# Tarseus/eam-rl4co

Hardware: AMD Instinct MI355X
Metric: env-steps/sec (batch x num_loc / s), AttentionModel construction rollout (higher is better)
Workload: dtype f32; 1 GPU; TSP num_loc=100 batch=1024/GPU AM greedy rollout (encoder + cache + decode loop + reward); global_batch=1024, launch=hipGraph replay

## Files before the change

eam_rl4co_amd/_lib.py:

```python
from __future__ import annotations

import ctypes as C
import os

_PKG = os.path.dirname(os.path.abspath(__file__))
LIB_PATH = os.environ.get("EAMRL_HIP_LIB") or os.path.join(_PKG, "lib", "libeamrl_hip.so")

ENV_TSP, ENV_CVRP, ENV_SDVRP, ENV_PCTSP, ENV_OP, ENV_CVRPTW, ENV_PDP = 0, 1, 2, 3, 4, 5, 6
GREEDY, SAMPLE, EVALUATE = 0, 1, 2
NORM_BATCH_EVAL, NORM_INSTANCE = 0, 1
ST_NAN_LOGITS, ST_INFEASIBLE, ST_STEP_OVERRUN = 1, 2, 4
LINEAR_NONE = 0

_vp, _i64, _i32, _f32 = C.c_void_p, C.c_int64, C.c_int, C.c_float


class Cache(C.Structure):
    _fields_ = [("K", _vp), ("V", _vp), ("Lp", _vp), ("Pa", _vp), ("Pb", _vp), ("cvec", _vp), ("gctx", _vp),
                ("ld", _i64), ("B", _i64), ("M", C.c_int32), ("E", C.c_int32), ("H", C.c_int32),
                ("dyn", _vp)]


class EncoderLayer(C.Structure):
    _fields_ = [(n, _vp) for n in ("Wqkv", "bqkv", "Wo", "bo", "W1", "b1", "W2", "b2", "n1_gamma", "n1_beta", "n1_mean",
                                   "n1_var", "n2_gamma", "n2_beta", "n2_mean", "n2_var")]


class EncoderCache(C.Structure):
    _fields_ = [("Wc", _vp), ("WoutT", _vp), ("out", _vp), ("ld", _i64), ("nproj", C.c_int32), ("Wg", _vp), ("gctx", _vp)]


class EncoderInit(C.Structure):
    _fields_ = [("feat", _vp), ("F", C.c_int32), ("W", _vp), ("b", _vp), ("depot", _vp), ("depot_ld", _i64), ("Wd", _vp),
                ("bd", _vp), ("init_out", _vp)]


class Reeval(C.Structure):
    _fields_ = [("K", _vp), ("V", _vp), ("Lp", _vp), ("Pa", _vp), ("Pb", _vp), ("ld", _i64),
                ("gctx", _vp), ("Cvec", _vp), ("NC", C.c_int32),
                ("idxA", _vp), ("idxB", _vp), ("sc", _vp), ("maskbits", _vp), ("actions", _vp),
                ("B", _i64), ("R", _i64), ("S", C.c_int32), ("T", C.c_int32), ("M", C.c_int32), ("tstart", C.c_int32),
                ("nchunk", C.c_int32), ("clip", _f32), ("temp", _f32),
                ("logp", _vp), ("lse", _vp), ("glogp", _vp), ("dheads", _vp), ("heads", _vp), ("heads_T", C.c_int32),
                ("entropy", _vp),
# ... 157 lines not shown
```

eam_rl4co_amd/csrc/abi.hip:

```cpp
#include <cstdarg>
#include <cstdio>

#include "kernels.hpp"


using namespace eamrl;

namespace eamrl { int g_debug[16] = {0}; }

static thread_local char g_err[256] = "";

static int fail(int code, const char* fmt, ...)
{
    va_list ap;
    va_start(ap, fmt);
    vsnprintf(g_err, sizeof(g_err), fmt, ap);
    va_end(ap);
    return code;
}

static int launched(int rc, const char* what)
{
    if (rc == 0) return 0;
    if (rc == EAMRL_E_ARG) return fail(rc, "%s: unsupported shape", what);
// ... 378 lines not shown
    REQUIRE(xy && code && out && R >= 0 && B > 0 && N > 0, "eamrl_augment_xy");
    REQUIRE(((uintptr_t)xy % 8 == 0) && ((uintptr_t)out % 8 == 0), "eamrl_augment_xy");
    return launched(launch_augment_xy(xy, cs, code, out, R, B, N, offset, (hipStream_t)stream), "eamrl_augment_xy");
}

static bool dtype16_ok(int dtype) { return dtype == EAMRL_DTYPE_F16 || dtype == EAMRL_DTYPE_BF16; }

static int encoder_fused_entry(const float* h_in, const eamrl_encoder_init* init, bool with_init, float* h_out, int64_t B, int M,
                               int E, int H, int ff_hidden, int nlayers, int norm, float eps, const eamrl_encoder_layer* layers,
                               const eamrl_encoder_cache* cache, int dtype, void* stream, const char* what)
{
    if (cache) {
        REQUIRE(cache->Wc && cache->WoutT && cache->out && cache->nproj >= 3 && cache->nproj <= 5, what);
        REQUIRE(cache->ld >= (int64_t)(cache->nproj + 1) * E && cache->ld % 4 == 0 && ((uintptr_t)cache->out % 16 == 0) &&
                    ((uintptr_t)cache->Wc % 16 == 0) && ((uintptr_t)cache->WoutT % 16 == 0), what);
    }
    REQUIRE(layers && B >= 0, what);
    REQUIRE(encoder_fused_supports(M, E, H, ff_hidden, nlayers), what);
    REQUIRE(norm == EAMRL_NORM_BATCH_EVAL || norm == EAMRL_NORM_INSTANCE, what);
    for (int l = 0; l < nlayers; ++l) {
        const eamrl_encoder_layer& s = layers[l];
        REQUIRE(s.Wqkv && s.bqkv && s.Wo && s.bo && s.W1 && s.b1 && s.W2 && s.b2 && s.n1_gamma && s.n1_beta && s.n2_gamma &&
                    s.n2_beta, what);
        REQUIRE(((uintptr_t)s.Wqkv % 16 == 0) && ((uintptr_t)s.Wo % 16 == 0) && ((uintptr_t)s.W1 % 16 == 0) &&
                    ((uintptr_t)s.W2 % 16 == 0), what);
        if (norm == EAMRL_NORM_BATCH_EVAL) REQUIRE(s.n1_mean && s.n1_var && s.n2_mean && s.n2_var, what);
    }
    if (with_init) {
        REQUIRE(init && init->feat && init->W && init->F >= 1 && init->F <= 8, what);
        REQUIRE(!init->depot || (init->Wd && init->depot_ld >= 2), what);
// ... 200 lines not shown
    REQUIRE(x && dy && mean && rstd && dx && B >= 0 && N > 0 && E > 0, "eamrl_instance_norm_backward");
    if (B == 0) return 0;
    return launched(launch_instnorm_train_bwd(x, dy, mean, rstd, gamma, dx, dgamma, dbeta, B, N, E, (hipStream_t)stream),
                    "eamrl_instance_norm_backward");
}

__attribute__((visibility("default"))) int eamrl_mean_nodes(const float* emb, float* out, int64_t B, int M, int E,
                                                           void* stream)
{
    REQUIRE(emb && out && B >= 0 && M > 0 && E > 0, "eamrl_mean_nodes");
    return launched(launch_mean_nodes(emb, out, B, M, E, (hipStream_t)stream), "eamrl_mean_nodes");
}

static int fill_args(const char* what, int env, const eamrl_cache* c, const eamrl_state* s, int64_t R, int mode,
                     const float* noise, const int64_t* given, float clip, float temp, int top_k, double top_p,
                     uint32_t* status, DecArgs& a, bool seeded = false)
{
    REQUIRE(c && s, what);
    REQUIRE(env >= EAMRL_ENV_TSP && env <= EAMRL_ENV_PDP, what);
    REQUIRE(mode == EAMRL_GREEDY || mode == EAMRL_SAMPLE || mode == EAMRL_EVALUATE, what);
    REQUIRE(c->K && c->V && c->Lp && c->Pa && (c->cvec || env == EAMRL_ENV_PDP), what);
    REQUIRE(c->B > 0 && c->M > 0 && c->E > 0 && c->H > 0, what);
    REQUIRE(c->E % c->H == 0 && (c->E / c->H) % 4 == 0 && c->E % (4 * EAMRL_NCHUNK) == 0, what);
    REQUIRE(c->ld >= c->E && c->ld % 4 == 0, what);
    REQUIRE(((uintptr_t)c->K % 16 == 0) && ((uintptr_t)c->V % 16 == 0) && ((uintptr_t)c->Lp % 16 == 0), what);
    REQUIRE(R > 0 && R % c->B == 0 && R <= 0x7fffffffLL, what);
    REQUIRE(s->cur && s->mask && status, what);
    REQUIRE(temp > 0.0f && top_k >= 0 && top_p >= 0.0 && top_p <= 1.0, what);
    if (env == EAMRL_ENV_TSP) REQUIRE(c->Pb && s->first && s->istep, what);
    if (env == EAMRL_ENV_CVRP) REQUIRE(s->used && s->vcap && c->M >= 2, what);
    if (env == EAMRL_ENV_SDVRP) REQUIRE(s->used && s->vcap && s->rem && c->dyn && c->M >= 2, what);
    if (env == EAMRL_ENV_PCTSP) REQUIRE(s->used && s->vcap && c->M >= 2, what);
    if (env == EAMRL_ENV_OP) REQUIRE(s->used && s->vcap && c->M >= 2, what);
    if (env == EAMRL_ENV_CVRPTW) REQUIRE(s->used && s->vcap && s->time && c->M >= 2, what);
    if (env == EAMRL_ENV_PDP) REQUIRE(c->M >= 3 && c->M % 2 == 1, what);
    if (mode == EAMRL_SAMPLE) REQUIRE(noise != nullptr || seeded, what);
    if (mode == EAMRL_EVALUATE) REQUIRE(given != nullptr, what);
    a = DecArgs{};
    a.K = c->K; a.V = c->V; a.Lp = c->Lp; a.Pa = c->Pa; a.Pb = c->Pb; a.cvec = c->cvec; a.gctx = c->gctx;
    a.ld = c->ld; a.B = c->B; a.M = c->M; a.E = c->E; a.H = c->H;
    a.first = s->first; a.cur = s->cur; a.istep = s->istep; a.used = s->used; a.vcap = s->vcap; a.demand = s->demand;
    a.mask = s->mask; a.visited = s->visited; a.done = s->done;
    a.rem = s->rem; a.dyn = c->dyn; a.locs = s->locs; a.time = s->time; a.tw = s->tw; a.dur = s->dur;
    a.heads_out = s->heads_out;
    a.to_deliver = s->to_deliver;
    a.seed = 0; a.seed_dev = nullptr; a.use_rng = 0;
    a.R = R; a.mode = mode; a.noise = noise; a.given = given; a.clip = clip; a.temp = temp; a.top_k = top_k; a.top_p = top_p; a.status = status;
    return 0;
}

__attribute__((visibility("default"))) int eamrl_am_decode_step(int env, const eamrl_cache* cache_host,
                                                               const eamrl_state* state_host, int64_t R, int mode,
                                                               const float* noise, const int64_t* given, float tanh_clip,
                                                               float temperature, int top_k, double top_p,
                                                               int fuse_env_step, int64_t* action,
                                                               float* logp, float* logprobs_all, float* logits_raw,
                                                               uint32_t* status, void* stream)
{
    DecArgs a;
    int rc = fill_args("eamrl_am_decode_step", env, cache_host, state_host, R, mode, noise, given, tanh_clip, temperature,
// ... 32 lines not shown
    DecArgs a{};
    a.B = cache_host->B; a.M = cache_host->M; a.E = cache_host->E; a.H = cache_host->H; a.ld = cache_host->ld; a.R = R;
    a.t_max = t_max; a.top_k = top_k; a.top_p = top_p;
    return rollout_kernel_for(env, a, true);
}

__attribute__((visibility("default"))) int eamrl_am_rollout(int env, const eamrl_cache* cache_host,
                                                           const eamrl_state* state_host, int64_t R, int mode,
                                                           const float* noise, const int64_t* given, int t_given,
                                                           float tanh_clip, float temperature, int top_k, double top_p,
                                                           int t_max, int64_t* actions, float* logps, int32_t* steps_out,
                                                           uint32_t* status, void* stream)
{
    DecArgs a;
    int rc = fill_args("eamrl_am_rollout", env, cache_host, state_host, R, mode, noise, given, tanh_clip, temperature,
                       top_k, top_p, status, a);
    if (rc) return rc;
    REQUIRE(actions && logps && steps_out && a.done && t_max > 0, "eamrl_am_rollout");
    if (env == EAMRL_ENV_CVRP) REQUIRE(a.visited && a.demand, "eamrl_am_rollout");
    if (env == EAMRL_ENV_PCTSP) REQUIRE(a.visited && a.demand && a.istep, "eamrl_am_rollout");
    if (env == EAMRL_ENV_OP) REQUIRE(a.visited && a.demand && a.istep && a.locs, "eamrl_am_rollout");
    if (env == EAMRL_ENV_CVRPTW) REQUIRE(a.visited && a.demand && a.locs && a.tw && a.dur, "eamrl_am_rollout");
    if (env == EAMRL_ENV_PDP) REQUIRE(a.visited && a.to_deliver, "eamrl_am_rollout");
    if (mode == EAMRL_EVALUATE) REQUIRE(t_given > 0, "eamrl_am_rollout");
    a.fuse_env = 1; a.t_max = t_max; a.t_given = t_given;
    a.action = actions; a.logp = logps; a.steps_out = steps_out;
    const int kernel = rollout_kernel_for(env, a, false);
    if (kernel == EAMRL_KERNEL_MS_MFMA)
        return launched(launch_rollout_ms_mfma(env, a, (hipStream_t)stream), "eamrl_am_rollout");
    if (kernel == EAMRL_KERNEL_RESIDENT)
        return launched(launch_rollout_resident(env, a, (hipStream_t)stream), "eamrl_am_rollout");
    return launched(launch_rollout_stream(env, a, (hipStream_t)stream), "eamrl_am_rollout");
}

__attribute__((visibility("default"))) int eamrl_exp1_noise(uint64_t seed, const uint64_t* seed_dev, float* noise, int64_t R,
                                                           int T, int M, void* stream)
{
    REQUIRE(noise && R >= 0 && T > 0 && M > 0, "eamrl_exp1_noise");
    return launched(launch_exp1_noise(seed, seed_dev, noise, R, T, M, (hipStream_t)stream), "eamrl_exp1_noise");
}

__attribute__((visibility("default"))) int eamrl_rollout_rng_native(int env, const eamrl_cache* cache_host, int64_t R)
// ... 1 lines not shown
    if (!cache_host || R <= 0 || g_debug[11]) return 0;
    DecArgs a{};
    a.B = cache_host->B; a.M = cache_host->M; a.E = cache_host->E; a.H = cache_host->H; a.ld = cache_host->ld; a.R = R;
    return rollout_ms_mfma_supports(env, a, true) ? 1 : 0;
}

__attribute__((visibility("default"))) int eamrl_am_rollout_seeded(int env, const eamrl_cache* cache_host,
                                                                  const eamrl_state* state_host, int64_t R, uint64_t seed,
                                                                  const uint64_t* seed_dev, float* noise_scratch,
                                                                  float tanh_clip, float temperature,
                                                                  int t_max, int64_t* actions, float* logps,
                                                                  int32_t* steps_out, uint32_t* status, void* stream)
{
    DecArgs a;
    int rc = fill_args("eamrl_am_rollout_seeded", env, cache_host, state_host, R, EAMRL_SAMPLE, nullptr, nullptr, tanh_clip,
                       temperature, 0, 0.0, status, a, true);
    if (rc) return rc;
    REQUIRE(actions && logps && steps_out && a.done && t_max > 0, "eamrl_am_rollout_seeded");
    a.fuse_env = 1; a.t_max = t_max; a.t_given = 0;
    a.action = actions; a.logp = logps; a.steps_out = steps_out;
    if (rollout_kernel_for(env, a, false) == EAMRL_KERNEL_MS_MFMA) {
        a.seed = seed; a.seed_dev = seed_dev; a.use_rng = 1;
        return launched(launch_rollout_ms_mfma(env, a, (hipStream_t)stream), "eamrl_am_rollout_seeded");
    }
    REQUIRE(noise_scratch != nullptr, "eamrl_am_rollout_seeded (noise_scratch [R][t_max][M] needed for this shape)");
    rc = launch_exp1_noise(seed, seed_dev, noise_scratch, R, t_max, a.M, (hipStream_t)stream);
    if (rc) return launched(rc, "eamrl_am_rollout_seeded");
    return eamrl_am_rollout(env, cache_host, state_host, R, EAMRL_SAMPLE, noise_scratch, nullptr, 0, tanh_clip, temperature, 0,
                            0.0, t_max, actions, logps, steps_out, status, stream);
}

static bool polynet_shape_ok(int env, const eamrl_cache* c, int64_t R)
{
    if (env != EAMRL_ENV_TSP && env != EAMRL_ENV_CVRP) return false;
    if (c->B <= 0 || R <= 0 || R % c->B != 0 || R > 0x7fffffffLL || R / c->B < 2) return false;
    DecArgs a{};
// ... 310 lines not shown
```

eam_rl4co_amd/csrc/decode_common.hpp:

```cpp
#pragma once
#include "../../include/eamrl.h"
#include "dmath.hpp"

namespace eamrl {

struct DecArgs {
    const float* K; const float* V; const float* Lp; const float* Pa; const float* Pb;
    const float* cvec; const float* gctx;
    int64_t ld; int64_t B; int M, E, H;
    int64_t* first; int64_t* cur; int64_t* istep; float* used; const float* vcap; const float* demand;
    uint8_t* mask; uint8_t* visited; uint8_t* done;
    float* rem; const float* dyn;
    const float* locs;
    float* time; const float* tw; const float* dur;
    int64_t R; int mode; const float* noise; const int64_t* given; int t_given;
    uint64_t seed; const uint64_t* seed_dev; int use_rng;
    float clip, temp; int fuse_env; int t_max;
    int top_k; double top_p;
    int64_t* action; float* logp; float* logprobs_all; float* logits_raw;
    int32_t* steps_out; uint32_t* status;
    float* heads_out;
    uint8_t* to_deliver;
};

struct RowLds {
    static constexpr int PAD = 4;
    float* q;
    float* heads;
    float* w;
    float* x;
    float* partA;
    float* partZ;
    float* partL;
    float* red;
    int* redi;
    uint8_t* msk;
};
// ... 27 lines not shown
```

eam_rl4co_amd/csrc/encoder_fused.hip:

```cpp
#include "encoder_fused.hpp"

namespace eamrl {

constexpr int SA = 140;
constexpr int GA = 34;
constexpr int SQ = 66;

struct ALayout {
    float* HB;
    static constexpr int S = SA;
    __device__ float* col(int c) const { return HB + (c & 3) * GA + (c >> 2); }
    __device__ void store4(int row, int q4, float4 v) const
    {
        float* p = HB + row * SA + q4;
        p[0] = v.x; p[GA] = v.y; p[2 * GA] = v.z; p[3 * GA] = v.w;
    }
    __device__ float4 load4(int row, int q4) const
    {
        const float* p = HB + row * SA + q4;
        return make_float4(p[0], p[GA], p[2 * GA], p[3 * GA]);
    }
    __device__ void mirror(int, int, float) const {}
};

// ... 447 lines not shown
    if (a.h_out) store_h(a.h_out, M, L);
    ESTAMP(13);
    const float* wpc[2];
    float4 bc[2];
    {
        const float* w0 = !a.cache.out ? a.L[0].Wqkv : a.cache.nproj == 0 ? a.cache.WoutT : a.cache.Wc;
#pragma unroll
        for (int ct = 0; ct < 2; ++ct) wpc[ct] = w0 + ((int64_t)(2 * cw + ct) * (FE / 16)) * 256 + lane * 4;
        load_b0<2>(bc, wpc);
    }
    if (a.cache.gctx) graph_context(a.cache.Wg, a.cache.gctx, M, L, CST);
    ESTAMP(19);
    if (a.cache.out) {
        float* STG = QA;
        float* crow = a.cache.out + (inst * (int64_t)M) * a.cache.ld;
        for (int sl = 0; sl <= a.cache.nproj; ++sl) {
            const bool lp = sl == a.cache.nproj;
            f32x4 acc[RTW][2];
#pragma unroll
            for (int ct = 0; ct < 2; ++ct)
#pragma unroll
                for (int rt = 0; rt < RTW; ++rt) acc[rt][ct] = splat4(0.0f);
            if (lp) __syncthreads();
            const float* arow = (lp ? STG : HB) + (row0 + j) * SA + G * GA;
            float2 a0[RTW][2];
            load_a0<RTW, SA>(a0, arow, nrt);
            gemm_pass<RTW, 2, SA, FE / 16, true, RTT - RTA>(acc, arow, nrt, wpc, bc, a0);
            {
                const int sn = lp ? sl : sl + 1;
#pragma unroll
                for (int ct = 0; ct < 2; ++ct)
                    wpc[ct] = (sn == a.cache.nproj ? a.cache.WoutT : a.cache.Wc + (int64_t)sn * FE * FE) +
                              ((int64_t)(2 * cw + ct) * (FE / 16)) * 256 + lane * 4;
                load_b0<2>(bc, wpc);
            }
#pragma unroll
            for (int rt = 0; rt < RTW; ++rt)
                if (rt < nrt) {
                    const int node = row0 + 16 * rt + j;
#pragma unroll
                    for (int ct = 0; ct < 2; ++ct) {
                        const int c = 32 * cw + 16 * ct + 4 * G;
                        const f32x4 v = acc[rt][ct];
                        if (node < M)
                            *reinterpret_cast<float4*>(crow + (int64_t)node * a.cache.ld + sl * FE + c) = make_float4(v[0], v[1], v[2], v[3]);
                        if (sl == 2) {
                            float* p = STG + node * SA + (c >> 2);
                            p[0] = v[0]; p[GA] = v[1]; p[2 * GA] = v[2]; p[3 * GA] = v[3];
                        }
                    }
                }
        }
    }
    ESTAMP(21);
#ifdef EAMRL_STAMPS
    if (lane == 0) {
        for (int i = 0; i < 22; ++i)
            if (i != 20) atomicAdd(&g_enc_stamps[i], st_acc[i]);
        atomicAdd(&g_enc_stamps[20], 1ull);
    }
#endif
}

__global__ void k_pack_mfma_b(const float* __restrict__ W, float* __restrict__ Wp, int N, int K)
{
    const int64_t idx = (int64_t)blockIdx.x * blockDim.x + threadIdx.x;
    if (idx >= (int64_t)N * K) return;
// ... 53 lines not shown
```

eam_rl4co_amd/csrc/encoder_fused16.hip:

```cpp
#include "encoder_fused.hpp"

namespace eamrl {
namespace {

constexpr int SH = 132;
constexpr int ST = 136;
constexpr int SQ = 72;

template <typename T> struct Mf;
template <> struct Mf<__bf16> {
    typedef __bf16 v8 __attribute__((ext_vector_type(8)));
    typedef __bf16 v4 __attribute__((ext_vector_type(4)));
    static __device__ __forceinline__ f32x4 k32(v8 a, v8 b, f32x4 c) { return __builtin_amdgcn_mfma_f32_16x16x32_bf16(a, b, c, 0, 0, 0); }
    static __device__ __forceinline__ f32x4 k16(v4 a, v4 b, f32x4 c) { return __builtin_amdgcn_mfma_f32_16x16x16bf16_1k(a, b, c, 0, 0, 0); }
};
template <> struct Mf<_Float16> {
    typedef _Float16 v8 __attribute__((ext_vector_type(8)));
    typedef _Float16 v4 __attribute__((ext_vector_type(4)));
    static __device__ __forceinline__ f32x4 k32(v8 a, v8 b, f32x4 c) { return __builtin_amdgcn_mfma_f32_16x16x32_f16(a, b, c, 0, 0, 0); }
    static __device__ __forceinline__ f32x4 k16(v4 a, v4 b, f32x4 c) { return __builtin_amdgcn_mfma_f32_16x16x16f16(a, b, c, 0, 0, 0); }
};

template <typename T>
__device__ __forceinline__ typename Mf<T>::v4 cvt4(float a, float b, float c, float d)
// ... 337 lines not shown
}

}

int launch_pack_mfma_b16(const float* W, void* Wp, int N, int K, int dtype, hipStream_t st)
{
    const int64_t n = (int64_t)N * K;
    const dim3 grid((unsigned)((n + 255) / 256));
    if (dtype == EAMRL_DTYPE_BF16) hipLaunchKernelGGL(k_pack16<__bf16>, grid, dim3(256), 0, st, W, (__bf16*)Wp, N, K);
    else hipLaunchKernelGGL(k_pack16<_Float16>, grid, dim3(256), 0, st, W, (_Float16*)Wp, N, K);
    return hipGetLastError() == hipSuccess ? 0 : EAMRL_E_LAUNCH;
}

int launch_encoder_fused16(const FusedArgs& a, int64_t B, int dtype, hipStream_t st)
{
    return dtype == EAMRL_DTYPE_BF16 ? launch16<__bf16>(a, B, st) : launch16<_Float16>(a, B, st);
}

}
```

eam_rl4co_amd/csrc/rollout_resident.hip:

```cpp
#include "kernels.hpp"
#include "env_rule.hpp"

namespace eamrl {

namespace {

constexpr int RB = 256;
constexpr int RE = 128;
constexpr int RH = 8;
constexpr int RD = 16;
constexpr int RNP = 128;
constexpr int RFM = 112;

bool res_filtering(const DecArgs& a) { return a.top_k > 0 || (a.top_p > 0.0 && a.top_p < 1.0); }

#ifdef EAMRL_STAMPS
__device__ unsigned long long g_stamps[8];
#define STAMP(i) do { if (wv == fw) { const unsigned long long now_ = __builtin_readcyclecounter(); \
                                     stamp_acc[i] += now_ - stamp_t; stamp_t = now_; } } while (0)
#else
#define STAMP(i) do { } while (0)
#endif

template <int CP, int TM, int SDF, int XYF, int TWF>
// ... 7 lines not shown
    float lp_out[TM];
    int16_t act_out[TM];
    float dynv[3 * SDF];
    float xy[2 * XYF];
    float twv[3 * TWF];
    int done;
    uint8_t msk[RNP];
    uint8_t vis[RNP];
};

constexpr int res_tmax(int env) { return (env == EAMRL_ENV_SDVRP ? 3 : 2) * RNP + 2; }
constexpr int res_sdf(int env) { return env == EAMRL_ENV_SDVRP ? RE : 4; }
constexpr int res_xyf(int env) { return (env == EAMRL_ENV_OP || env == EAMRL_ENV_CVRPTW) ? RNP : 2; }
constexpr int res_twf(int env) { return env == EAMRL_ENV_CVRPTW ? RNP : 2; }

template <int ENV, int CP, int CR, bool MS, bool FILT>
__global__ __launch_bounds__(RB, 2) void k_rollout_resident(DecArgs a, int S, int G)
{
    constexpr bool SD = ENV == EAMRL_ENV_SDVRP;
    constexpr bool PC = ENV == EAMRL_ENV_PCTSP;
    constexpr bool OP = ENV == EAMRL_ENV_OP;
    constexpr bool TW = ENV == EAMRL_ENV_CVRPTW;
    constexpr bool CV = ENV == EAMRL_ENV_CVRP || TW;
    constexpr bool PD = ENV == EAMRL_ENV_PDP;
    extern __shared__ __attribute__((aligned(16))) char smem[];
    using L = ResLds<CP, res_tmax(ENV), res_sdf(ENV), res_xyf(ENV), res_twf(ENV)>;
    L& l = *reinterpret_cast<L*>(smem);
    float* Plds = reinterpret_cast<float*>(smem + ((sizeof(L) + 15) & ~size_t(15)));
    constexpr int WROW = L::WROW;

    const int tid = threadIdx.x, lane = tid & 63, wv = tid >> 6;
    const int ve = 32 * wv + (lane & 31), vg = lane >> 5;
    const int M = a.M;
    const int64_t bi = blockIdx.x % a.B;
    const int64_t ld = a.ld;
    const int C = (M + EAMRL_NCHUNK - 1) / EAMRL_NCHUNK;
    const int n0 = lane, n1 = lane + 64;
    const bool in0 = n0 < M, in1 = n1 < M;

// ... 84 lines not shown
    if (wv == fw) {
        cur = a.cur[r];
        if (ENV == EAMRL_ENV_TSP) { first = a.first[r]; istep = a.istep[r]; }
        else if (PD) {
            pvis[0] = __ballot(in0 && a.visited[r * M + (in0 ? n0 : 0)] != 0);
            pvis[1] = __ballot(in1 && a.visited[r * M + (in1 ? n1 : 0)] != 0);
            ptd[0] = __ballot(in0 && a.to_deliver[r * M + (in0 ? n0 : 0)] != 0);
            ptd[1] = __ballot(in1 && a.to_deliver[r * M + (in1 ? n1 : 0)] != 0);
        }
        else { used = a.used[r]; vcap = a.vcap[r]; }
        if (PC || OP) { istep = a.istep[r]; i0 = istep; }
        if (TW) now = a.time[r];
        const int c0 = (ENV == EAMRL_ENV_TSP) ? (in0 && l.msk[n0] != 0) : (in0 && l.vis[n0] != 0 && !(PC && n0 == 0));
        const int c1 = (ENV == EAMRL_ENV_TSP) ? (in1 && l.msk[n1] != 0) : (in1 && l.vis[n1] != 0);
        count = __builtin_popcountll(__ballot(c0)) + __builtin_popcountll(__ballot(c1));
#pragma unroll
        for (int k = 0; k < 2; ++k) {
            const int e = lane + 64 * k;
            gq[k] = a.gctx ? a.gctx[bi * RE + e] : 0.0f;
            cv[k] = PD ? 0.0f : a.cvec[e];
            if (ENV == EAMRL_ENV_TSP && istep > 0) p1f[k] = a.Pa[(bi * M + first) * ld + e];
            const int nn = lane + 64 * k;
            if (CV && nn >= 1 && nn < M) mydem[k] = l.dem[nn - 1];
            float ctx;
            if (ENV == EAMRL_ENV_TSP) ctx = (istep == 0) ? cv[k] : p1f[k] + Plds[cur * RE + e];
            else if (PC) ctx = fma_(cv[k], (vcap - used) < 0.0f ? 0.0f : (vcap - used), Plds[cur * RE + e]);
            else ctx = fma_(cv[k], vcap - used, Plds[cur * RE + e]);
            if (TW) { cv2[k] = a.cvec[RE + e]; ctx = fma_(cv2[k], now, ctx); }
            l.q[e] = ctx + gq[k];
        }
    }
    __syncthreads();

    int t = 0;
    uint32_t st_flags = 0;
#ifdef EAMRL_STAMPS
// ... 261 lines not shown
            sel = __builtin_amdgcn_readfirstlane(sel);
            if (__ballot(nan_seen) != 0ull) st_flags |= EAMRL_ST_NAN_LOGITS;
            if (sel < 0 || sel >= M) { st_flags |= EAMRL_ST_INFEASIBLE; sel = 0; }
            const bool sel_ok = (((sel < 64) ? (fb0 >> sel) : (fb1 >> (sel - 64))) & 1ull) != 0ull;
            if (!sel_ok) st_flags |= EAMRL_ST_INFEASIBLE;
            const float lp_sel = __int_as_float(
                (sel < 64) ? __builtin_amdgcn_readlane(__float_as_int(lpv[0]), sel)
                           : __builtin_amdgcn_readlane(__float_as_int(lpv[1]), sel - 64));
            if (lane == 0) {
                l.act_out[t] = (int16_t)sel;
                l.lp_out[t] = lp_sel;
            }
            if (ENV == EAMRL_ENV_TSP) {
                if (istep == 0) {
                    first = sel;
#pragma unroll
                    for (int k = 0; k < 2; ++k) p1f[k] = a.Pa[(bi * M + first) * ld + lane + 64 * k];
                }
                cur = sel;
                istep += 1;
                count -= sel_ok ? 1 : 0;
                done = (count == 0);
                __builtin_amdgcn_wave_barrier();
                if (lane == 0) { l.msk[sel] = 0; l.done = done; }
#pragma unroll
                for (int k = 0; k < 2; ++k) l.q[lane + 64 * k] = (p1f[k] + Plds[cur * RE + lane + 64 * k]) + gq[k];
            } else if (OP) {
                const float cx = l.xy[2 * sel], cy = l.xy[2 * sel + 1];
                used = used + rule::leg(cx, cy, l.xy[2 * cur], l.xy[2 * cur + 1]);
                done = rule::tour_ends(sel == 0, istep);
                cur = sel;
                istep += 1;
// ... 164 lines not shown
{
    const size_t lds = ((sizeof(ResLds<CP, res_tmax(ENV), res_sdf(ENV), res_xyf(ENV), res_twf(ENV)>) + 15) & ~size_t(15)) +
                       (size_t)a.M * RE * sizeof(float) + (FILT ? 2 * RNP * sizeof(float) : 0);
    auto k = k_rollout_resident<ENV, CP, CR, MS, FILT>;
    if (lds > 64 * 1024 &&
        hipFuncSetAttribute(reinterpret_cast<const void*>(k), hipFuncAttributeMaxDynamicSharedMemorySize, (int)lds) != hipSuccess)
        return EAMRL_E_LAUNCH;
    hipLaunchKernelGGL(k, dim3((unsigned)(MS ? a.B * G : a.R)), dim3(RB), lds, st, a, S, G);
    return 0;
}

template <int ENV, int CP, int CR, bool FILT>
int launch_cp(const DecArgs& a, hipStream_t st)
{
    const int64_t S = a.R / a.B;
    int rc;
    if (S > 1 && a.R % a.B == 0 && !g_debug[6]) {
        int64_t G = (4 * 512 + a.B - 1) / a.B;
        G = G < 1 ? 1 : (G > S ? S : G);
        rc = launch_ms<ENV, CP, CR, true, FILT>(a, (int)S, (int)G, st);
    } else {
        rc = launch_ms<ENV, CP, CR, false, FILT>(a, 1, 1, st);
    }
    if (rc) return rc;
    launch_rollout_pad(ENV, a, st);
    return hipGetLastError() == hipSuccess ? 0 : EAMRL_E_LAUNCH;
}

template <int ENV>
int launch_env(const DecArgs& a, hipStream_t st)
// ... 48 lines not shown
```

eam_rl4co_amd/ops.py:

```python
from __future__ import annotations

import ctypes as C
import logging
import os

import torch

from . import _lib, env_spec
from ._lib import (ENV_CVRP, ENV_CVRPTW, ENV_OP, ENV_PCTSP, ENV_PDP, ENV_SDVRP, ENV_TSP, EVALUATE, GREEDY, NORM_BATCH_EVAL, NORM_INSTANCE, SAMPLE,
                   ST_INFEASIBLE, ST_NAN_LOGITS, ST_STEP_OVERRUN)

MODES = {"greedy": GREEDY, "sampling": SAMPLE, "evaluate": EVALUATE}
ENVS = {name: spec.abi_id for name, spec in env_spec.ENV_SPECS.items()}


def _need_gpu(t: torch.Tensor, name: str):
    if not t.is_cuda:
        raise RuntimeError(
            f"{name} is on {t.device}: the eam_rl4co_amd rollout path runs only on an MI355X (HIP) device; "
            "there is no CPU fallback. Move the TensorDict / policy to 'cuda'.")


def _chk(t, name, dtype, shape=None):
    if not isinstance(t, torch.Tensor):
# ... 406 lines not shown
    arr = (_lib.EncoderLayer * len(layers))()
    for i, d in enumerate(layers):
        for name, _ in _lib.EncoderLayer._fields_:
            t = d.get(name)
            if t is not None:
                _need_gpu(t, name)
                want = wdt if name in _PACKED_FIELDS else torch.float32
                if t.dtype != want or not t.is_contiguous():
                    raise TypeError(f"{what}: {name} must be contiguous {want}")
            setattr(arr[i], name, _ptr(t))
    out = torch.empty(B, M, E, dtype=torch.float32, device=dev) if (store_hidden or cache is None) else None
    cstruct = None
    if cache is not None:
        Wc, WoT, buf, nproj = cache[:4]
        Wg, gctx = cache[4:6] if len(cache) >= 6 else (None, None)
        _chk(Wc, "packed cache weights", wdt, (nproj * E * E,))
        _chk(WoT, "packed project_out^T", wdt, (E * E,))
        _chk(buf, "decoder cache", torch.float32)
        if buf.dim() != 3 or buf.shape[0] != B or buf.shape[1] != M or buf.shape[2] < (nproj + 1) * E:
            raise ValueError(f"{what}: cache buffer must be [B, M, >= (nproj + 1) * E]")
        cs = _lib.EncoderCache()
        cs.Wc, cs.WoutT, cs.out, cs.ld, cs.nproj = _ptr(Wc), _ptr(WoT), _ptr(buf), buf.shape[2], int(nproj)
        if Wg is not None:
            _chk(Wg, "project_fixed_context.weight", torch.float32, (E, E))
            _chk(gctx, "graph context", torch.float32, (B, E))
            if Wg.data_ptr() % 16:
                raise ValueError(f"{what}: Wg must be 16-byte aligned")
            cs.Wg, cs.gctx = _ptr(Wg), _ptr(gctx)
        cstruct = C.byref(cs)
    if init is not None:
        ist = _lib.EncoderInit()
        b, depot, Wd, bd = init.get("b"), init.get("depot"), init.get("Wd"), init.get("bd")
        for name, t in (("init_embed.bias", b), ("depot", depot), ("init_embed_depot.weight", Wd), ("init_embed_depot.bias", bd)):
            if t is not None:
                _need_gpu(t, name)
                if t.dtype != torch.float32:
                    raise TypeError(f"{what}: {name} must be fp32")
# ... 785 lines not shown
                                      M - 1, L, G, float(mutation_rate), float(crossover_rate), float(selection_rate),
                                      int(bool(top_k)), _ptr(init_mut_rand), _ptr(init_mut_u), nul(cross_rand),
                                      nul(cross_u), nul(mut_rand), nul(mut_u), _stream(pop)), "eamrl_ea_prize_run")
    return fitness


class DecodeCache:

    def __init__(self, env_name, buf, cvec, gctx, embeddings, num_heads, dyn=None, embed_dim=None):
        self.env_name, self.buf, self.cvec, self.gctx = env_name, buf, cvec, gctx
        self.dyn = dyn
        self.node_embeddings = embeddings
        self.E = embeddings.shape[-1] if embeddings is not None else int(embed_dim)
        self.H = num_heads
        self.slots = slot_map(env_name)
        self.planes = buf.dim() == 4
        if self.planes:
            P, self.B, self.M, self.ld = buf.shape
            assert P == len(self.slots) and self.ld == self.E
        else:
            self.B, self.M, self.ld = buf.shape
            assert self.ld == len(self.slots) * self.E

    def view(self, name):
        i = self.slots[name]
        return self.buf[i] if self.planes else self.buf[..., i * self.E:(i + 1) * self.E]

    @property
    def glimpse_key(self):
        return self.view("K")
# ... 9 lines not shown
    @property
    def graph_context(self):
        return self.gctx if self.gctx is not None else 0

    def struct(self):
        c = _lib.Cache()
        base, step = self.buf.data_ptr(), (self.B * self.M * self.E * 4 if self.planes else self.E * 4)
        c.K = C.c_void_p(base + self.slots["K"] * step)
        c.V = C.c_void_p(base + self.slots["V"] * step)
        c.Lp = C.c_void_p(base + self.slots["Lp"] * step)
        c.Pa = C.c_void_p(base + self.slots["Pa"] * step)
        c.Pb = C.c_void_p(base + self.slots["Pb"] * step) if "Pb" in self.slots else None
        c.cvec, c.gctx = _ptr(self.cvec), _ptr(self.gctx)
        c.ld, c.B, c.M, c.E, c.H = self.ld, self.B, self.M, self.E, self.H
        c.dyn = _ptr(self.dyn)
        return c


def slot_map(env_name):
    names = ["K", "V", "L", "Pa", "Pb", "Lp"] if env_spec.ENV_SPECS[env_name].has_pb else ["K", "V", "L", "Pa", "Lp"]
    return {n: i for i, n in enumerate(names)}


class RolloutState:
    first = cur = istep = used = vcap = demand = mask = visited = done = rem = locs = time = tw = dur = None
    heads_out = to_deliver = None

    def __init__(self, env_name, R, M, device, demand=None):
        self.env_name, self.R, self.M = env_name, R, M
        self.done = torch.zeros(R, dtype=torch.bool, device=device)
# ... 415 lines not shown
```

eam_rl4co_amd/policy.py:

```python
from __future__ import annotations

import logging
import os
from typing import Optional

import torch
import torch.nn as nn

from . import ops
from .env_spec import ACTION, ALIASES, ENV_SPECS, max_steps
from .envs import ENV_REGISTRY, RL4COEnvBase, get_env
from .tensordict_lite import TensorDict
from .utils import unbatchify, unbatchify_and_gather

log = logging.getLogger(__name__)

DECODE_TYPES = ("greedy", "sampling", "multistart_greedy", "multistart_sampling", "evaluate")

PRECISIONS = {"32-true": None, "16-mixed": torch.float16, "bf16-mixed": torch.bfloat16}


def _kind(env_name):
    if isinstance(env_name, RL4COEnvBase):
        env_name = env_name.name
# ... 206 lines not shown
                                      for _ in range(num_layers)))
        self.dtype16 = None

    def forward(self, x, mask=None, cache_spec=None, init=None, store_hidden=True, fused=None):
        assert mask is None, "Mask not yet supported!"
        if fused is None:
            assert init is None, "init= needs the fused kernel (check _fused_layers first)"
            fused = self._fused_layers(x)
        if fused is not None:
            layers, H, ff, norm, eps, dtype = fused
            cache = None
            if cache_spec is not None:
                if cache_spec.get("dtype") != dtype:
                    raise RuntimeError("fused encoder: the decoder cache spec was packed for another precision")
                cache = (cache_spec["Wc"], cache_spec["WoT"], cache_spec["buf"], cache_spec["nproj"], cache_spec.get("Wg"),
                         cache_spec.get("gctx"))
            h = None if init is not None else x.contiguous()
            if dtype is None:
                out = ops.encoder_fused(h, layers, H, ff, norm, eps, cache=cache, init=init, store_hidden=store_hidden)
            else:
                out = ops.encoder_fused16(h, layers, H, ff, norm, eps, dtype, cache=cache, init=init, store_hidden=store_hidden)
            if cache_spec is not None:
                cache_spec["filled"] = True
            return out
        for layer in self.layers:
            x = layer(x)
        return x

    def _fused_layers(self, x, shape=None):
        if os.environ.get("EAMRL_FUSED_ENCODER", "1") == "0" or len(self.layers) == 0:
            return None
# ... 588 lines not shown
        ent = None
        if want_ent:
            re, ent = re
            ent = ent.sum(1)
        td_mask = p["td"].get("mask", None) if hasattr(p["td"], "get") else None
        if td_mask is not None:
            re = re.masked_fill(~td_mask, 0)
        if p["return_sum_log_likelihood"]:
            re = re.sum(1)
        out = dict(out)
        out["log_likelihood"] = out["log_likelihood"].detach() + (re - re.detach())
        if ent is not None:
            out["entropy"] = out["entropy"].detach() + (ent - ent.detach())
        return out

    def _enqueue(self, td, env, phase, calc_reward, return_actions, return_entropy, return_hidden, return_init_embeds,
                 return_sum_log_likelihood, actions, max_steps, **decoding_kwargs) -> dict:
        if isinstance(env, str) or env is None:
            env = get_env(self.env_alias if env is None else env)
        if _kind(env.name) != self.env_name:
            raise ValueError(f"policy built for {self.env_alias!r} got env {env.name!r}")

        decode_type = decoding_kwargs.pop("decode_type", None)
        given_type = None
        if actions is not None:
            given_type, decode_type = decode_type, "evaluate"
        elif decode_type is None:
            decode_type = getattr(self, f"{phase}_decode_type")
        if decode_type == "beam_search":
            return {"out": self._beam_search(td, env, decoding_kwargs, calc_reward, return_actions,
# ... 32 lines not shown
            multisample = num_samples > 1
        if num_starts is not None:
            multistart = num_starts > 1
        S = 0
        if multistart or multisample:
            S = num_starts if multistart else num_samples
            if S is None:
                S = env.get_num_starts(td)
        mode = "evaluate" if actions is not None else ("greedy" if "greedy" in decode_type else "sampling")

        spec = None
        if isinstance(self.encoder, AttentionModelEncoder) and isinstance(self.decoder, AttentionModelDecoder):
            Bq, Mq = td["action_mask"].shape
            spec = self.decoder._fused_cache_spec(Bq, Mq, td["action_mask"].device, dtype=self._dtype16)
        shared, ekey, ent = getattr(self, "_shared_dt", None), None, None
        if shared is not None and spec is not None:
            from .train import _graph_key

            ekey = _graph_key(self, td)
            ent = shared.get("native")
            ent = ent if ent is not None and ent[0] == ekey else None
        if ent is not None:
            hidden, init_embeds, spec = ent[1:]
            if init_embeds is None and return_init_embeds:
                init_embeds = self.encoder.init_embedding(td)
        else:
            if spec is not None and isinstance(self.encoder, AttentionModelEncoder):
                need_emb = (return_hidden or ekey is not None
                            or (self.decoder.use_graph_context and spec.get("gctx") is None))
                hidden, init_embeds = self.encoder(td, cache_spec=spec, want_hidden=need_emb, want_init=return_init_embeds)
            else:
                hidden, init_embeds = self.encoder(td, cache_spec=spec) if spec is not None else self.encoder(td)
            if ekey is not None and spec.get("filled"):
                shared["native"] = (ekey, hidden, init_embeds, spec)
        cache = self.decoder._precompute_cache(hidden, num_starts=S, prefilled=spec)

        st = state_from_td(self.env_name, td, S)
        pre_actions, pre_logps = [], []
        if S >= 1 and multistart:
            if actions is not None:
                start, actions = actions[..., 0].contiguous(), actions[..., 1:]
            elif select_start_nodes_fn is not None:
                start = select_start_nodes_fn(td, env, S)
            else:
                start = env.select_start_nodes(td, num_starts=S)
            start = start.to(torch.int64).contiguous()
            _env_step_(st, start)
            pre_actions, pre_logps = [start[:, None]], [torch.zeros(st.R, 1, dtype=torch.float32, device=start.device)]

        M = st.M
# ... 526 lines not shown
```

include/eamrl.h:

```cpp
#ifndef EAMRL_H
#define EAMRL_H

#include <stdint.h>

#ifdef __cplusplus
extern "C" {
#endif

#define EAMRL_VERSION 101

#define EAMRL_ENV_TSP 0
#define EAMRL_ENV_CVRP 1
#define EAMRL_ENV_SDVRP 2
#define EAMRL_ENV_PCTSP 3
#define EAMRL_ENV_OP 4
#define EAMRL_ENV_CVRPTW 5
#define EAMRL_ENV_PDP 6
#define EAMRL_GREEDY 0
#define EAMRL_SAMPLE 1
#define EAMRL_EVALUATE 2
#define EAMRL_NORM_BATCH_EVAL 0
#define EAMRL_NORM_INSTANCE 1
#define EAMRL_DTYPE_F16 1
#define EAMRL_DTYPE_BF16 2
// ... 124 lines not shown
    const float* b1;
    const float* W2;
    const float* b2;
    const float *n1_gamma, *n1_beta, *n1_mean, *n1_var;
    const float *n2_gamma, *n2_beta, *n2_mean, *n2_var;
} eamrl_encoder_layer;

typedef struct eamrl_encoder_cache {
    const float* Wc;
    const float* WoutT;
    float* out;
    int64_t ld;
    int nproj;
    const float* Wg;
    float* gctx;
} eamrl_encoder_cache;

typedef struct eamrl_encoder_init {
    const float* feat;
    int F;
    const float* W;
    const float* b;
    const float* depot;
    int64_t depot_ld;
    const float* Wd;
    const float* bd;
    float* init_out;
} eamrl_encoder_init;

int eamrl_pack_linear_weight(const float* W, float* Wp, int out_dim, int in_dim, void* stream);
// ... 58 lines not shown
int eamrl_tsp_mask_bits_chunked(const int64_t* actions, uint32_t* bits, int64_t R, int M, int T, void* stream);


typedef struct eamrl_cache {
    const float* K;
    const float* V;
    const float* Lp;
    const float* Pa;
    const float* Pb;
    const float* cvec;
    const float* gctx;
    int64_t ld;
    int64_t B;
    int32_t M, E, H;
    const float* dyn;
} eamrl_cache;

typedef struct eamrl_state {
    int64_t* first;
    int64_t* cur;
    int64_t* istep;
    float* used;
    const float* vcap;
    const float* demand;
    uint8_t* mask;
    uint8_t* visited;
    uint8_t* done;
    float* rem;
    const float* locs;
    float* time;
// ... 155 lines not shown
```

Before: 51.02 million env-steps/s.

## Skip unused decoder-cache projections in encoder epilogue for lean TSP greedy rollout

In the fused encoder's cache epilogue, adds bitmasks that skip storing the logit-key slot and skip the GEMM for the first-node projection slot, writing raw hidden embeddings there instead. The resident TSP rollout kernel then computes the first-node projection on the fly from the raw hidden row and the weight matrix, once per rollout. This is meant to cut encoder epilogue GEMM work and cache write bandwidth, in exchange for a per-row dot product in the decoder and extra validation and gating logic restricted to single-start f32 TSP on the resident kernel.

```diff
diff --git a/eam_rl4co_amd/_lib.py b/eam_rl4co_amd/_lib.py
--- a/eam_rl4co_amd/_lib.py
+++ b/eam_rl4co_amd/_lib.py
@@ -18,7 +18,7 @@
 class Cache(C.Structure):
     _fields_ = [("K", _vp), ("V", _vp), ("Lp", _vp), ("Pa", _vp), ("Pb", _vp), ("cvec", _vp), ("gctx", _vp),
                 ("ld", _i64), ("B", _i64), ("M", C.c_int32), ("E", C.c_int32), ("H", C.c_int32),
-                ("dyn", _vp)]
+                ("dyn", _vp), ("Wa", _vp), ("pa_raw", C.c_int32)]
 
 
 class EncoderLayer(C.Structure):
@@ -27,7 +27,8 @@
 
 
 class EncoderCache(C.Structure):
-    _fields_ = [("Wc", _vp), ("WoutT", _vp), ("out", _vp), ("ld", _i64), ("nproj", C.c_int32), ("Wg", _vp), ("gctx", _vp)]
+    _fields_ = [("Wc", _vp), ("WoutT", _vp), ("out", _vp), ("ld", _i64), ("nproj", C.c_int32), ("Wg", _vp), ("gctx", _vp),
+                ("skip_store", C.c_uint32), ("raw_h", C.c_uint32)]
 
 
 class EncoderInit(C.Structure):
diff --git a/eam_rl4co_amd/csrc/abi.hip b/eam_rl4co_amd/csrc/abi.hip
--- a/eam_rl4co_amd/csrc/abi.hip
+++ b/eam_rl4co_amd/csrc/abi.hip
@@ -416,6 +416,9 @@
         REQUIRE(cache->Wc && cache->WoutT && cache->out && cache->nproj >= 3 && cache->nproj <= 5, what);
         REQUIRE(cache->ld >= (int64_t)(cache->nproj + 1) * E && cache->ld % 4 == 0 && ((uintptr_t)cache->out % 16 == 0) &&
                     ((uintptr_t)cache->Wc % 16 == 0) && ((uintptr_t)cache->WoutT % 16 == 0), what);
+        REQUIRE((cache->skip_store >> (cache->nproj + 1)) == 0, what);
+        REQUIRE((cache->raw_h & ~(((1u << cache->nproj) - 1u) & ~7u)) == 0 && (cache->raw_h & cache->skip_store) == 0, what);
+        REQUIRE(dtype == DTYPE_F32 || (cache->skip_store == 0 && cache->raw_h == 0), what);
     }
     REQUIRE(layers && B >= 0, what);
     REQUIRE(encoder_fused_supports(M, E, H, ff_hidden, nlayers), what);
@@ -646,7 +649,7 @@
 
 static int fill_args(const char* what, int env, const eamrl_cache* c, const eamrl_state* s, int64_t R, int mode,
                      const float* noise, const int64_t* given, float clip, float temp, int top_k, double top_p,
-                     uint32_t* status, DecArgs& a, bool seeded = false)
+                     uint32_t* status, DecArgs& a, bool seeded = false, bool raw_ok = false)
 {
     REQUIRE(c && s, what);
     REQUIRE(env >= EAMRL_ENV_TSP && env <= EAMRL_ENV_PDP, what);
@@ -668,6 +671,8 @@
     if (env == EAMRL_ENV_PDP) REQUIRE(c->M >= 3 && c->M % 2 == 1, what);
     if (mode == EAMRL_SAMPLE) REQUIRE(noise != nullptr || seeded, what);
     if (mode == EAMRL_EVALUATE) REQUIRE(given != nullptr, what);
+    REQUIRE(c->pa_raw == 0 || (raw_ok && c->pa_raw == 1 && env == EAMRL_ENV_TSP && R == c->B && c->Wa &&
+                               (uintptr_t)c->Wa % 16 == 0 && (uintptr_t)c->Pa % 16 == 0), what);
     a = DecArgs{};
     a.K = c->K; a.V = c->V; a.Lp = c->Lp; a.Pa = c->Pa; a.Pb = c->Pb; a.cvec = c->cvec; a.gctx = c->gctx;
     a.ld = c->ld; a.B = c->B; a.M = c->M; a.E = c->E; a.H = c->H;
@@ -676,6 +681,7 @@
     a.rem = s->rem; a.dyn = c->dyn; a.locs = s->locs; a.time = s->time; a.tw = s->tw; a.dur = s->dur;
     a.heads_out = s->heads_out;
     a.to_deliver = s->to_deliver;
+    a.Wa = c->Wa; a.pa_raw = c->pa_raw;
     a.seed = 0; a.seed_dev = nullptr; a.use_rng = 0;
     a.R = R; a.mode = mode; a.noise = noise; a.given = given; a.clip = clip; a.temp = temp; a.top_k = top_k; a.top_p = top_p; a.status = status;
     return 0;
@@ -738,7 +744,7 @@
 {
     DecArgs a;
     int rc = fill_args("eamrl_am_rollout", env, cache_host, state_host, R, mode, noise, given, tanh_clip, temperature,
-                       top_k, top_p, status, a);
+                       top_k, top_p, status, a, false, true);
     if (rc) return rc;
     REQUIRE(actions && logps && steps_out && a.done && t_max > 0, "eamrl_am_rollout");
     if (env == EAMRL_ENV_CVRP) REQUIRE(a.visited && a.demand, "eamrl_am_rollout");
@@ -750,6 +756,7 @@
     a.fuse_env = 1; a.t_max = t_max; a.t_given = t_given;
     a.action = actions; a.logp = logps; a.steps_out = steps_out;
     const int kernel = rollout_kernel_for(env, a, false);
+    REQUIRE(!a.pa_raw || kernel == EAMRL_KERNEL_RESIDENT, "eamrl_am_rollout");
     if (kernel == EAMRL_KERNEL_MS_MFMA)
         return launched(launch_rollout_ms_mfma(env, a, (hipStream_t)stream), "eamrl_am_rollout");
     if (kernel == EAMRL_KERNEL_RESIDENT)
@@ -781,12 +788,13 @@
 {
     DecArgs a;
     int rc = fill_args("eamrl_am_rollout_seeded", env, cache_host, state_host, R, EAMRL_SAMPLE, nullptr, nullptr, tanh_clip,
-                       temperature, 0, 0.0, status, a, true);
+                       temperature, 0, 0.0, status, a, true, true);
     if (rc) return rc;
     REQUIRE(actions && logps && steps_out && a.done && t_max > 0, "eamrl_am_rollout_seeded");
     a.fuse_env = 1; a.t_max = t_max; a.t_given = 0;
     a.action = actions; a.logp = logps; a.steps_out = steps_out;
     if (rollout_kernel_for(env, a, false) == EAMRL_KERNEL_MS_MFMA) {
+        REQUIRE(!a.pa_raw, "eamrl_am_rollout_seeded");
         a.seed = seed; a.seed_dev = seed_dev; a.use_rng = 1;
         return launched(launch_rollout_ms_mfma(env, a, (hipStream_t)stream), "eamrl_am_rollout_seeded");
     }
diff --git a/eam_rl4co_amd/csrc/decode_common.hpp b/eam_rl4co_amd/csrc/decode_common.hpp
--- a/eam_rl4co_amd/csrc/decode_common.hpp
+++ b/eam_rl4co_amd/csrc/decode_common.hpp
@@ -21,6 +21,7 @@
     int32_t* steps_out; uint32_t* status;
     float* heads_out;
     uint8_t* to_deliver;
+    const float* Wa; int pa_raw;
 };
 
 struct RowLds {
diff --git a/eam_rl4co_amd/csrc/encoder_fused.hip b/eam_rl4co_amd/csrc/encoder_fused.hip
--- a/eam_rl4co_amd/csrc/encoder_fused.hip
+++ b/eam_rl4co_amd/csrc/encoder_fused.hip
@@ -485,8 +485,11 @@
     if (a.cache.out) {
         float* STG = QA;
         float* crow = a.cache.out + (inst * (int64_t)M) * a.cache.ld;
-        for (int sl = 0; sl <= a.cache.nproj; ++sl) {
+        const unsigned skip = a.cache.skip_store, raw = a.cache.raw_h;
+        for (int sl = 0, sn; sl <= a.cache.nproj; sl = sn) {
             const bool lp = sl == a.cache.nproj;
+            sn = sl + 1;
+            while (sn < a.cache.nproj && ((raw >> sn) & 1u)) ++sn;
             f32x4 acc[RTW][2];
 #pragma unroll
             for (int ct = 0; ct < 2; ++ct)
@@ -498,13 +501,14 @@
             load_a0<RTW, SA>(a0, arow, nrt);
             gemm_pass<RTW, 2, SA, FE / 16, true, RTT - RTA>(acc, arow, nrt, wpc, bc, a0);
             {
-                const int sn = lp ? sl : sl + 1;
+                const int sw = lp ? sl : sn;
 #pragma unroll
                 for (int ct = 0; ct < 2; ++ct)
-                    wpc[ct] = (sn == a.cache.nproj ? a.cache.WoutT : a.cache.Wc + (int64_t)sn * FE * FE) +
+                    wpc[ct] = (sw == a.cache.nproj ? a.cache.WoutT : a.cache.Wc + (int64_t)sw * FE * FE) +
                               ((int64_t)(2 * cw + ct) * (FE / 16)) * 256 + lane * 4;
                 load_b0<2>(bc, wpc);
             }
+            const bool keep = ((skip >> sl) & 1u) == 0;
 #pragma unroll
             for (int rt = 0; rt < RTW; ++rt)
                 if (rt < nrt) {
@@ -513,7 +517,7 @@
                     for (int ct = 0; ct < 2; ++ct) {
                         const int c = 32 * cw + 16 * ct + 4 * G;
                         const f32x4 v = acc[rt][ct];
-                        if (node < M)
+                        if (keep && node < M)
                             *reinterpret_cast<float4*>(crow + (int64_t)node * a.cache.ld + sl * FE + c) = make_float4(v[0], v[1], v[2], v[3]);
                         if (sl == 2) {
                             float* p = STG + node * SA + (c >> 2);
@@ -522,6 +526,12 @@
                     }
                 }
         }
+        for (int sr = 3; sr < a.cache.nproj; ++sr)
+            if ((raw >> sr) & 1u)
+                for (int idx = tid; idx < M * (FE / 4); idx += 512) {
+                    const int row = idx / (FE / 4), q4 = idx % (FE / 4);
+                    *reinterpret_cast<float4*>(crow + (int64_t)row * a.cache.ld + sr * FE + 4 * q4) = L.load4(row, q4);
+                }
     }
     ESTAMP(21);
 #ifdef EAMRL_STAMPS
diff --git a/eam_rl4co_amd/csrc/encoder_fused16.hip b/eam_rl4co_amd/csrc/encoder_fused16.hip
--- a/eam_rl4co_amd/csrc/encoder_fused16.hip
+++ b/eam_rl4co_amd/csrc/encoder_fused16.hip
@@ -375,6 +375,7 @@
 
 int launch_encoder_fused16(const FusedArgs& a, int64_t B, int dtype, hipStream_t st)
 {
+    if (a.cache.out && (a.cache.skip_store || a.cache.raw_h)) return EAMRL_E_ARG;
     return dtype == EAMRL_DTYPE_BF16 ? launch16<__bf16>(a, B, st) : launch16<_Float16>(a, B, st);
 }
 
diff --git a/eam_rl4co_amd/csrc/rollout_resident.hip b/eam_rl4co_amd/csrc/rollout_resident.hip
--- a/eam_rl4co_amd/csrc/rollout_resident.hip
+++ b/eam_rl4co_amd/csrc/rollout_resident.hip
@@ -45,6 +45,25 @@
 constexpr int res_xyf(int env) { return (env == EAMRL_ENV_OP || env == EAMRL_ENV_CVRPTW) ? RNP : 2; }
 constexpr int res_twf(int env) { return env == EAMRL_ENV_CVRPTW ? RNP : 2; }
 
+__device__ __forceinline__ void pa_first_from_h(const float* __restrict__ hrow, const float* __restrict__ Wa, int lane, float (&p)[2])
+{
+    typedef const __attribute__((address_space(1))) f32x4m* gptr;
+    const char* hb = reinterpret_cast<const char*>(hrow);
+    const char* wb = reinterpret_cast<const char*>(Wa);
+    asm volatile("" : "+v"(lane));
+    const unsigned off = (unsigned)lane * (RE * 4u);
+    float a0 = 0.0f, a1 = 0.0f;
+#pragma unroll 2
+    for (unsigned k = 0; k < RE * 4u; k += 16u) {
+        const f32x4m x = *(gptr)(hb + k), u = *(gptr)(wb + k + off), v = *(gptr)(wb + 64 * RE * 4 + k + off);
+        a0 = __builtin_fmaf(x[0], u[0], a0); a1 = __builtin_fmaf(x[0], v[0], a1);
+        a0 = __builtin_fmaf(x[1], u[1], a0); a1 = __builtin_fmaf(x[1], v[1], a1);
+        a0 = __builtin_fmaf(x[2], u[2], a0); a1 = __builtin_fmaf(x[2], v[2], a1);
+        a0 = __builtin_fmaf(x[3], u[3], a0); a1 = __builtin_fmaf(x[3], v[3], a1);
+    }
+    p[0] = a0; p[1] = a1;
+}
+
 template <int ENV, int CP, int CR, bool MS, bool FILT>
 __global__ __launch_bounds__(RB, 2) void k_rollout_resident(DecArgs a, int S, int G)
 {
@@ -54,6 +73,7 @@
     constexpr bool TW = ENV == EAMRL_ENV_CVRPTW;
     constexpr bool CV = ENV == EAMRL_ENV_CVRP || TW;
     constexpr bool PD = ENV == EAMRL_ENV_PDP;
+    constexpr bool RAWPA = ENV == EAMRL_ENV_TSP && !MS;
     extern __shared__ __attribute__((aligned(16))) char smem[];
     using L = ResLds<CP, res_tmax(ENV), res_sdf(ENV), res_xyf(ENV), res_twf(ENV)>;
     L& l = *reinterpret_cast<L*>(smem);
@@ -168,12 +188,16 @@
         const int c0 = (ENV == EAMRL_ENV_TSP) ? (in0 && l.msk[n0] != 0) : (in0 && l.vis[n0] != 0 && !(PC && n0 == 0));
         const int c1 = (ENV == EAMRL_ENV_TSP) ? (in1 && l.msk[n1] != 0) : (in1 && l.vis[n1] != 0);
         count = __builtin_popcountll(__ballot(c0)) + __builtin_popcountll(__ballot(c1));
+        if constexpr (RAWPA) {
+            if (a.pa_raw && istep > 0)
+                pa_first_from_h(a.Pa + (bi * M + __builtin_amdgcn_readfirstlane((int)first)) * ld, a.Wa, lane, p1f);
+        }
 #pragma unroll
         for (int k = 0; k < 2; ++k) {
             const int e = lane + 64 * k;
             gq[k] = a.gctx ? a.gctx[bi * RE + e] : 0.0f;
             cv[k] = PD ? 0.0f : a.cvec[e];
-            if (ENV == EAMRL_ENV_TSP && istep > 0) p1f[k] = a.Pa[(bi * M + first) * ld + e];
+            if (ENV == EAMRL_ENV_TSP && istep > 0 && !(RAWPA && a.pa_raw)) p1f[k] = a.Pa[(bi * M + first) * ld + e];
             const int nn = lane + 64 * k;
             if (CV && nn >= 1 && nn < M) mydem[k] = l.dem[nn - 1];
             float ctx;
@@ -465,8 +489,12 @@
             if (ENV == EAMRL_ENV_TSP) {
                 if (istep == 0) {
                     first = sel;
-#pragma unroll
-                    for (int k = 0; k < 2; ++k) p1f[k] = a.Pa[(bi * M + first) * ld + lane + 64 * k];
+                    if (RAWPA && a.pa_raw) {
+                        pa_first_from_h(a.Pa + (bi * M + sel) * ld, a.Wa, lane, p1f);
+                    } else {
+#pragma unroll
+                        for (int k = 0; k < 2; ++k) p1f[k] = a.Pa[(bi * M + first) * ld + lane + 64 * k];
+                    }
                 }
                 cur = sel;
                 istep += 1;
@@ -661,6 +689,7 @@
 int launch_cp(const DecArgs& a, hipStream_t st)
 {
     const int64_t S = a.R / a.B;
+    if (a.pa_raw && (ENV != EAMRL_ENV_TSP || a.R != a.B || !a.Wa)) return EAMRL_E_ARG;
     int rc;
     if (S > 1 && a.R % a.B == 0 && !g_debug[6]) {
         int64_t G = (4 * 512 + a.B - 1) / a.B;
diff --git a/eam_rl4co_amd/ops.py b/eam_rl4co_amd/ops.py
--- a/eam_rl4co_amd/ops.py
+++ b/eam_rl4co_amd/ops.py
@@ -444,6 +444,7 @@
     if cache is not None:
         Wc, WoT, buf, nproj = cache[:4]
         Wg, gctx = cache[4:6] if len(cache) >= 6 else (None, None)
+        skip_store, raw_h = (int(cache[6] or 0), int(cache[7] or 0)) if len(cache) >= 8 else (0, 0)
         _chk(Wc, "packed cache weights", wdt, (nproj * E * E,))
         _chk(WoT, "packed project_out^T", wdt, (E * E,))
         _chk(buf, "decoder cache", torch.float32)
@@ -451,6 +452,7 @@
             raise ValueError(f"{what}: cache buffer must be [B, M, >= (nproj + 1) * E]")
         cs = _lib.EncoderCache()
         cs.Wc, cs.WoutT, cs.out, cs.ld, cs.nproj = _ptr(Wc), _ptr(WoT), _ptr(buf), buf.shape[2], int(nproj)
+        cs.skip_store, cs.raw_h = skip_store, raw_h
         if Wg is not None:
             _chk(Wg, "project_fixed_context.weight", torch.float32, (E, E))
             _chk(gctx, "graph context", torch.float32, (B, E))
@@ -1266,6 +1268,7 @@
         self.E = embeddings.shape[-1] if embeddings is not None else int(embed_dim)
         self.H = num_heads
         self.slots = slot_map(env_name)
+        self.pa_raw_Wa = None
         self.planes = buf.dim() == 4
         if self.planes:
             P, self.B, self.M, self.ld = buf.shape
@@ -1305,6 +1308,8 @@
         c.cvec, c.gctx = _ptr(self.cvec), _ptr(self.gctx)
         c.ld, c.B, c.M, c.E, c.H = self.ld, self.B, self.M, self.E, self.H
         c.dyn = _ptr(self.dyn)
+        if self.pa_raw_Wa is not None:
+            c.Wa, c.pa_raw = _ptr(self.pa_raw_Wa), 1
         return c
 
 
diff --git a/eam_rl4co_amd/policy.py b/eam_rl4co_amd/policy.py
--- a/eam_rl4co_amd/policy.py
+++ b/eam_rl4co_amd/policy.py
@@ -244,7 +244,7 @@
                 if cache_spec.get("dtype") != dtype:
                     raise RuntimeError("fused encoder: the decoder cache spec was packed for another precision")
                 cache = (cache_spec["Wc"], cache_spec["WoT"], cache_spec["buf"], cache_spec["nproj"], cache_spec.get("Wg"),
-                         cache_spec.get("gctx"))
+                         cache_spec.get("gctx"), cache_spec.get("skip_store", 0), cache_spec.get("raw_h", 0))
             h = None if init is not None else x.contiguous()
             if dtype is None:
                 out = ops.encoder_fused(h, layers, H, ff, norm, eps, cache=cache, init=init, store_hidden=store_hidden)
@@ -863,6 +863,18 @@
             out["entropy"] = out["entropy"].detach() + (ent - ent.detach())
         return out
 
+    def _lean_cache_ok(self, spec, S, multistart, max_steps, top_k, top_p, kept) -> bool:
+        if kept or spec.get("dtype") is not None or os.environ.get("EAMRL_LEAN_CACHE", "1") == "0":
+            return False
+        if type(self.decoder) is not AttentionModelDecoder or self._pointer_operands() is not None:
+            return False
+        B, M, ld = spec["buf"].shape
+        shape = ops._lib.Cache()
+        shape.B, shape.M, shape.E, shape.H, shape.ld = B, M, self.decoder.embed_dim, self.decoder.num_heads, ld
+        t_max = _max_decode_steps(self.env_name, M, 1 if (S >= 1 and multistart) else 0)
+        t_max = int(max(1, min(t_max, max_steps)))
+        return B > 0 and ops.rollout_kernel(self.env_name, shape, B * max(S, 1), t_max, top_k, top_p) == "resident"
+
     def _enqueue(self, td, env, phase, calc_reward, return_actions, return_entropy, return_hidden, return_init_embeds,
                  return_sum_log_likelihood, actions, max_steps, **decoding_kwargs) -> dict:
         if isinstance(env, str) or env is None:
@@ -925,6 +937,15 @@
             Bq, Mq = td["action_mask"].shape
             spec = self.decoder._fused_cache_spec(Bq, Mq, td["action_mask"].device, dtype=self._dtype16)
         shared, ekey, ent = getattr(self, "_shared_dt", None), None, None
+        pa_raw = False
+        if spec is not None and shared is None and self._lean_cache_ok(
+                spec, S, multistart, max_steps, top_k, top_p,
+                kept=return_hidden or entropy_native or store_all_logp or bool(getattr(self, "_want_heads", False))):
+            slots = ops.slot_map(self.env_name)
+            spec["skip_store"] = 1 << slots["L"]
+            pa_raw = self.env_name == "tsp" and S == 0
+            if pa_raw:
+                spec["raw_h"] = 1 << slots["Pa"]
         if shared is not None and spec is not None:
             from .train import _graph_key
 
@@ -945,6 +966,8 @@
             if ekey is not None and spec.get("filled"):
                 shared["native"] = (ekey, hidden, init_embeds, spec)
         cache = self.decoder._precompute_cache(hidden, num_starts=S, prefilled=spec)
+        if pa_raw and spec.get("filled"):
+            cache.pa_raw_Wa = self.decoder._weight_constants()[0]
 
         st = state_from_td(self.env_name, td, S)
         pre_actions, pre_logps = [], []
diff --git a/include/eamrl.h b/include/eamrl.h
--- a/include/eamrl.h
+++ b/include/eamrl.h
@@ -162,6 +162,8 @@
     int nproj;
     const float* Wg;
     float* gctx;
+    uint32_t skip_store;
+    uint32_t raw_h;
 } eamrl_encoder_cache;
 
 typedef struct eamrl_encoder_init {
@@ -250,6 +252,8 @@
     int64_t B;
     int32_t M, E, H;
     const float* dyn;
+    const float* Wa;
+    int32_t pa_raw;
 } eamrl_cache;
 
 typedef struct eamrl_state {
```

Result: no change. 51.05 million env-steps/s (median of 3 runs) (+0.1%).
